# Shanmuk4622/RL-Project-Heist-Architect-Adversarial-Reinforcement-Learning-Framework-CSE4019

Hardware: AMD Instinct MI355X
Metric: Solver env-steps/sec at 20×20, 4096 envs/GPU, 1/2/4/8 MI355X (higher is better)
Workload: dtype f64

## Files before the change

rl-project-heist-architect-adversarial-reinforcement-learning-framework-cse4019_amd/csrc/heist_env.hip:

```cpp
#include <type_traits>
#include <utility>

#include "heist_device.h"
#include "heist_fan_intervals.h"
#include "heist_trig.h"

#pragma clang fp contract(off)

namespace heist {

__constant__ double kSinCosTab[4 * HEIST_SINCOS_TAB_ROWS] = HEIST_SINCOS_TAB_INIT;
constexpr int kTabDoubles = 4 * HEIST_SINCOS_TAB_ROWS;

__device__ __forceinline__ int iabs_(int a) { return a < 0 ? -a : a; }
__device__ __forceinline__ int unpack_r(uint16_t v) { return v & 0xff; }
__device__ __forceinline__ int unpack_c(uint16_t v) { return v >> 8; }

__device__ __forceinline__ double py_mod360(double x) {
  if (x > 0.0 && x < 720.0) return x >= 360.0 ? x - 360.0 : x;
  double r = fmod(x, 360.0);
  if (r != 0.0) {
    if (r < 0.0) r += 360.0;
  } else {
    r = 0.0;
// ... 1976 lines not shown
  float2* uq = reinterpret_cast<float2*>(reinterpret_cast<unsigned char*>(tb) + align16(sizeof(TieBuckets)));
  const int n_chunk = (RC + 63) >> 6;
  const int nvis = (RC + 31) >> 5, WR = (nvis + 4) & ~3;
  uint16_t* togo = reinterpret_cast<uint16_t*>(uq + 128 * W);
  uint32_t* vrow = reinterpret_cast<uint32_t*>(togo + 2 * RC);
  const EnvBase eb = env_base(p, e);

  {
    EmitterRaw raw;
    prefetch<NT>(p, e, eb, L, raw);
    if (t < n_slot) rec[t] = raw;
  }
  for (int i = t; i < path_words; i += NT) L.path[i] = eb.paths[i];
  for (int i = t; i < (int)sizeof(TieBuckets) / 4; i += NT)
    reinterpret_cast<uint32_t*>(tb)[i] = reinterpret_cast<const uint32_t*>(&kTieBuckets_)[i];
  const EnvScalars s = p.scal[e];
  const int tick0 = uni(s.tick);
  int HK = p.max_steps - tick0;
  HK = HK < H ? HK : H;
  if (uni(s.done) || HK < 0) HK = 0;
  const int g = t - mc;
  const bool live_cam = t < s.n_cams, live_guard = g >= 0 && g < s.n_guards;
  bool cached = false;
  uint4 ca = make_uint4(0u, 0u, 0u, 0u), cb = ca;
  auto next_entry = [&](const Guard& gd) {
    int idx = gd.idx, slot = gd.hslot;
    if (gd.len >= 2) {
      idx += gd.step;
      if (idx >= gd.len) idx -= gd.len;
      slot = gd.nslot;
    }
    const uint4* src = reinterpret_cast<const uint4*>(eb.cones + cone_off(g, idx, slot));
    ca = src[0];
    cb = src[1];
  };
  auto take_entry = [&]() {
    Guard gd = as_guard(rec[t]);
    gd.nslot = (uint8_t)(cb.w >> 16);
    rec[t] = __builtin_bit_cast(EmitterRaw, gd);
    uint4* dst = reinterpret_cast<uint4*>(L.cone + 16 * g);
    dst[0] = ca;
    dst[1] = cb;
  };
  __syncthreads();
  if (HK > 0 && live_guard) {
    const Guard gd = as_guard(rec[t]);
    cached = gd.hslot != kUncached;
    if (cached) next_entry(gd);
  }

  const uint32_t cdiv = ((1u << 20) + (uint32_t)C - 1u) / (uint32_t)C;

  for (int k = 1; k <= HK; ++k) {
    Emit E;
    E.kind = -1;
    if (w0) {
      if (live_cam) {
        Cam cm = as_cam(rec[t]);
        cm.heading = py_mod360(cm.heading + cm.speed * 1.0);
        rec[t] = __builtin_bit_cast(EmitterRaw, cm);
        E = cam_emit(cm);
      } else if (live_guard) {
        Guard gd = as_guard(rec[t]);
        const bool moves = gd.len >= 2;
        int nidx = gd.idx;
        if (moves) {
          nidx += gd.step;
          if (nidx >= gd.len) nidx -= gd.len;
        }
        const uint16_t np = moves ? L.path[__umul24((uint32_t)g, (uint32_t)p.max_path) + (uint32_t)nidx] : gd.pos;
        if (cached) {
          if (moves) gd.hslot = gd.nslot;
        } else if (moves) {
          gd.heading = guard_heading_after(p, unpack_r(np) - unpack_r(gd.pos), unpack_c(np) - unpack_c(gd.pos),
                                           gd.heading);
        }
        gd.idx = (int16_t)nidx;
        gd.pos = np;
        rec[t] = __builtin_bit_cast(EmitterRaw, gd);
        E = guard_emit(gd);
        if (cached && !SOLO) take_entry();
      }
      publish_emitters(L, E, n_slot);
    }
    clear_planes<NT>(p, L, gvis, true);
    __syncthreads();
    if (live_guard && E.kind == 1) L.vis[L.at(E.row, E.col)] = 1;
    cast_rays<NT, D, false, true>(smem, L, p.ray_mode, 0, p.half_deg, tb, uq);
    if (SOLO && cached) take_entry();
    stamp_guard_cones<NT>(L, gvis, mc, mg, 0);
    __syncthreads();

    uint32_t* row = vis_out + ((size_t)(k - 1) * N + e) * WR;
    for (int ch = wave; ch < n_chunk; ch += W) {
      const int cell = 64 * ch + lane;
      bool on = false;
      if (cell < RC) {
        const int r = (int)(((uint32_t)cell * cdiv) >> 20), c = cell - r * C;
        const int a = L.at(r, c);
        on = (L.vis[a] | gvis[a]) != 0;
      }
      const unsigned long long m = __ballot(on);
      if (lane < 2 && 2 * ch + lane < WR) row[2 * ch + lane] = (uint32_t)(m >> (32 * lane));
    }
    for (int i = 2 * n_chunk + t; i < WR; i += NT) row[i] = 0u;
    if (w0 && live_guard && cached && k < HK) next_entry(as_guard(rec[t]));
    __syncthreads();
  }

  {
    const int q4 = WR >> 2;
    const uint4 z = make_uint4(0u, 0u, 0u, 0u);
    for (int i = t; i < (H - HK) * q4; i += NT) {
      const int r = HK + i / q4, q = i - (i / q4) * q4;
      reinterpret_cast<uint4*>(vis_out + ((size_t)r * N + e) * WR)[q] = z;
    }
  }
  if (togo_ticks_out)
    for (int k = HK; k < H; ++k) {
      int16_t* trow = togo_ticks_out + ((size_t)k * N + e) * RC;
      for (int x = t; x < RC; x += NT) trow[x] = (int16_t)-1;
    }
  if (HK == 0) {
    for (int x = t; x < RC; x += NT) {
      togo_out[(size_t)e * RC + x] = (int16_t)-1;
      action_out[(size_t)e * RC + x] = (int8_t)-1;
    }
    return;
  }

  __threadfence();
  for (int x = t; x < RC; x += NT) togo[(HK & 1) * RC + x] = (uint16_t)kNone;
  auto load_row = [&](int k) {
    return __hip_atomic_load(vis_out + ((size_t)k * N + e) * WR + (t < nvis ? t : 0), __ATOMIC_RELAXED,
                             __HIP_MEMORY_SCOPE_AGENT);
  };
  __syncthreads();
  {
    const uint32_t w = load_row(HK - 1);
    if (t < nvis) vrow[((HK - 1) & 1) * nvis + t] = w;
  }
  __syncthreads();
  const int vcell = p.vr * C + p.vc;
  for (int k = HK - 1; k >= 0; --k) {
    uint32_t ahead = 0u;
    if (k > 0) ahead = load_row(k - 1);
    const uint32_t* vk = vrow + (k & 1) * nvis;
    const uint16_t* nxt = togo + ((k + 1) & 1) * RC;
    uint16_t* cur = togo + (k & 1) * RC;
    int16_t* trow = togo_ticks_out ? togo_ticks_out + ((size_t)k * N + e) * RC : nullptr;
    for (int x = t; x < RC; x += NT) {
      uint32_t best = kNone;
      int act = -1;
      if (L.grid[x] != kWall) {
        const int r = (int)(((uint32_t)x * cdiv) >> 20), c = x - r * C;
        auto val = [&](int y) -> uint32_t {
          if ((vk[y >> 5] >> (y & 31)) & 1u) return kNone;
          if (y == vcell) return 1u;
          const uint32_t v = nxt[y];
          return v == kNone ? kNone : v + 1u;
        };
        auto moved = [&](bool inside, int y) { return inside && L.grid[y] != kWall ? y : x; };
        best = val(x);
        act = 0;
        uint32_t v = val(moved(r > 0, x - C));
        if (v < best) best = v, act = 1;
        v = val(moved(r + 1 < p.R, x + C));
        if (v < best) best = v, act = 2;
        v = val(moved(c > 0, x - 1));
        if (v < best) best = v, act = 3;
        v = val(moved(c + 1 < C, x + 1));
        if (v < best) best = v, act = 4;
        if (best == kNone) act = -1;
      }
      cur[x] = (uint16_t)best;
      if (trow) trow[x] = (int16_t)(uint16_t)best;
      if (k == 0) {
        togo_out[(size_t)e * RC + x] = (int16_t)(uint16_t)best;
        action_out[(size_t)e * RC + x] = (int8_t)act;
      }
    }
    if (k > 0 && t < nvis) vrow[((k - 1) & 1) * nvis + t] = ahead;
    __syncthreads();
  }
}


__device__ __forceinline__ void lds_dma16(const void* gsrc, uint32_t lds_dst) {
  unsigned keep;
  asm volatile("s_mov_b32 %0, m0\n\ts_mov_b32 m0, %2\n\ts_nop 0\n\tglobal_load_lds_dwordx4 %1, off\n\ts_mov_b32 m0, %0"
               : "=&s"(keep)
               : "v"(gsrc), "s"(lds_dst)
               : "memory");
}

template <int D, int PC>
__device__ __noinline__ void lean_tie_rays(unsigned char* smem, const FanTick* f, int n_tie, uint32_t cam_rc, int n_cams,
                                           const double* hd) {
  const int lane = threadIdx.x;
  for (int b0 = 0; b0 < n_tie; b0 += 64) {
    const int tr = b0 + lane < n_tie ? (int)f->tie[b0 + lane] : -1;
    for (int m = 0; m < n_cams; ++m) {
      Emit E;
      E.hmh = f->hmh;
      E.fov = f->fov;
      E.step = 0.0;
      E.range = f->range;
      E.num_rays = f->num_rays;
      const uint32_t rcm = (uint32_t)__builtin_amdgcn_readlane((int)cam_rc, m);
      E.row = (int)(rcm & 0xffu);
      E.col = (int)(rcm >> 8);
      E.first = 0;
      E.kind = 0;
      E.members = 1;
      if (tr >= 0) exact_ray<D>(smem, E, tr, PC, 0, hd);
    }
  }
}

template <int D, int PC>
__device__ __noinline__ void ivl_tie_rays(unsigned char* smem, int ray, double hmh, double fov, int num_rays,
                                          uint32_t rc, const double* hd) {
  Emit E;
  E.hmh = hmh;
  E.fov = fov;
  E.step = 0.0;
  E.range = kTieMaxRange;
  E.num_rays = num_rays;
  E.row = (int)(rc & 0xffu);
  E.col = (int)(rc >> 8);
  E.first = 0;
  E.kind = 0;
  E.members = 1;
  if (ray >= 0) exact_ray<D>(smem, E, ray, PC, 0, hd);
}

size_t step_multi_lds(const EnvParams& p, int K);
struct LeanStage {
  uint4 off4[128];
  uint2 off2[128];
  int hdr[4];
};

constexpr double kFanUnitsPerDeg = 4294967296.0 / 360.0;
struct IvlTable {
  uint32_t cut[kFanCuts];
  float2 dir[kFanCuts];
  uint8_t idx[368];
};
static_assert(sizeof(IvlTable) % 16 == 0, "copied in 16-byte words");
constexpr IvlTable make_ivl_table() {
  IvlTable t{};
  for (int j = 0; j < kFanCuts; ++j) {
    t.cut[j] = kFanCut[j];
    t.dir[j] = float2{kFanDir[j][0], kFanDir[j][1]};
  }
  for (int d = 0; d < 361; ++d) t.idx[d] = kFanIdx[d];
  return t;
}
__constant__ IvlTable kIvlTable = make_ivl_table();
constexpr size_t kLeanUnion = sizeof(LeanStage) > sizeof(IvlTable) ? sizeof(LeanStage) : sizeof(IvlTable);
struct LeanLds {
  uint8_t* grid;
  uint16_t* path;
  uint8_t* act;
  LeanStage* stg;
  IvlTable* ivl;
  uint4* icam;
  int32_t* icim;
  uint16_t* cone;
  uint16_t* rcone;
  uint8_t* gpl;
  float4* plane2;
};
__host__ __device__ constexpr int lean_gap(int R, int C) { return (R + 2 * kRing) * (C + 2 * kRing) <= 1024 ? 1024 : 2048; }
__host__ __device__ inline size_t lean_carve(unsigned char* smem, int R, int C, int mc, int mg, int mp, int K,
                                             LeanLds* L) {
  size_t o = 3 * (size_t)lean_gap(R, C);
  if (L) L->grid = smem + o;
  o += align16((size_t)R * C);
  if (L) L->path = reinterpret_cast<uint16_t*>(smem + o);
  o += align16(2 * (size_t)mg * mp);
  if (L) L->act = smem + o;
  o += align16((size_t)K);
  if (L) L->stg = reinterpret_cast<LeanStage*>(smem + o);
  if (L) L->ivl = reinterpret_cast<IvlTable*>(smem + o);
  o += align16(kLeanUnion);
  if (L) L->icam = reinterpret_cast<uint4*>(smem + o);
  o += 16 * (size_t)(mc > 0 ? mc : 1);
  if (L) L->icim = reinterpret_cast<int32_t*>(smem + o);
  o += align16(8 * (size_t)(mc > 0 ? mc : 1));
  if (L) L->cone = reinterpret_cast<uint16_t*>(smem + o);
  o += 64 * (size_t)(mg > 0 ? mg : 1);
  if (L) L->rcone = reinterpret_cast<uint16_t*>(smem + o);
  o += 64 * (size_t)(mg > 0 ? mg : 1);
  if (L) L->gpl = smem + o;
  o += align16((size_t)R * C);
  if (L) L->plane2 = reinterpret_cast<float4*>(smem + o);
  o += 4 * (size_t)R * C;
  return o;
}
static size_t lean_lds_bytes(const EnvParams& p, int K) {
  const size_t lean = align16(lean_carve(nullptr, p.R, p.C, p.max_cams, p.max_guards, p.max_path, K, nullptr)) +
                      (p.stamps ? 80 : 0);
  const size_t generic = step_multi_lds(p, K);
  return lean > generic ? lean : generic;
}


struct LeanGuard {
  uint32_t a, b, nslot;
  __device__ int idx() const { return (int)(a & 0xffu); }
  __device__ int step() const { return (int)((a >> 8) & 0xffu); }
  __device__ int len() const { return (int)((a >> 16) & 0xffu); }
  __device__ int hslot() const { return (int)(a >> 24); }
  __device__ uint32_t pos() const { return b & 0xffffu; }
  __device__ uint32_t pos0() const { return b >> 16; }
};

template <int D, bool REC>
__device__ __attribute__((noinline)) void lean_generic_body(EnvParams p, int K, const int64_t* __restrict__ actions,
                                                            obs_out_t<REC>* __restrict__ obs, float* __restrict__ rew,
                                                            double* __restrict__ rew64, uint8_t* __restrict__ done_out,
                                                            int8_t* __restrict__ status_out, int auto_reset,
                                                            unsigned char* smem, int e) {
  step_multi_body<1, D, false, 0, REC>(p, K, actions, obs, rew, rew64, done_out, status_out, auto_reset, smem, e);
}

template <int R_, int C_, bool STAMP = false, int NW = 1, bool REC = false>
__global__ __launch_bounds__(64 * NW) __attribute__((amdgpu_waves_per_eu(4))) void step_lean_kernel(
    EnvParams p, int K, const int64_t* __restrict__ actions, obs_out_t<REC>* __restrict__ obs, float* __restrict__ rew,
    double* __restrict__ rew64, uint8_t* __restrict__ done_out, int8_t* __restrict__ status_out, int auto_reset) {
  constexpr int D = lean_gap(R_, C_);
  constexpr int PC = C_ + 2 * kRing;
  constexpr int RC = R_ * C_;
  constexpr int N4 = RC / 4;
  constexpr int C4 = C_ / 4;
  constexpr int Q = (N4 + 63) / 64;
  constexpr int OFF0 = kRing * PC + kRing;
  static_assert((R_ + 2 * kRing) * PC <= D, "the padded planes fit the 1024-byte gap");
  static_assert(C_ % 4 == 0 && R_ <= 64 && C_ <= 32 && (R_ + 2 * kRing) * PC <= 2048, "lean kernel geometry");
  static_assert(NW == 1 || (NW == 2 && !STAMP && Q % 2 == 0), "two waves: the plain form, even Q");
  constexpr int QW = Q / NW;
  static_assert(!REC || !STAMP, "record output: the plain instances only");
  constexpr int NVIS = (RC + 31) / 32;
  constexpr int RW = (NVIS + 1 + 3) & ~3;
  constexpr int kStores = REC ? QW + 1 + 4 : 3 * QW + 4;
  extern __shared__ __align__(16) unsigned char smem[];
  const int e = block_env(p);
  if (p.prio_mode && p.dispatch_order) {
    const int pr = (int)((uint32_t)p.order[blockIdx.x] >> 24);
    if (pr == 3) __builtin_amdgcn_s_setprio(3);
    else if (pr == 2) __builtin_amdgcn_s_setprio(2);
    else if (pr == 1) __builtin_amdgcn_s_setprio(1);
  }
  const int lane = NW == 1 ? (int)threadIdx.x : (int)(threadIdx.x & 63u);
  const int wid = NW == 1 ? 0 : __builtin_amdgcn_readfirstlane((int)(threadIdx.x >> 6));
  const int tid = threadIdx.x;
  const int N = p.n_envs;
  const int mc = p.max_cams, mg = p.max_guards, n_slot = mc + mg, mp = p.max_path;
  const EnvBase eb = env_base(p, e);
  const FanTick* fan0 = p.fan + p.fan_base;

  EnvScalars s = p.scal[e];
  const int g = lane - mc;
  double heading = 0.0, speed = 0.0;
  uint32_t cam_rc = 0;
  LeanGuard gd{0u, 0u, 0u};
  const bool live_cam = lane < s.n_cams, live_guard = g >= 0 && g < s.n_guards;
  bool cached = false;
  double fovd = 0.0, su = 1.0;
  int32_t im_fx = 0;
  int cam_n = 0;
  bool ivl = false;
  {
    EmitterRaw rec;
    rec.a = make_uint4(0u, 0u, 0u, 0u);
    rec.b = rec.a;
    if (lane < n_slot) {
      const uint4* rs = lane < mc ? reinterpret_cast<const uint4*>(eb.cams + (uint32_t)lane)
                                  : reinterpret_cast<const uint4*>(eb.guards + (uint32_t)g);
      rec.a = rs[0];
      rec.b = rs[1];
    }
    const Cam cm = as_cam(rec);
    const Guard gr = as_guard(rec);
    heading = cm.heading;
    speed = cm.speed;
    cam_rc = (uint32_t)cm.row | ((uint32_t)cm.col << 8);
    cached = live_guard && gr.hslot != kUncached;
    gd.a = (uint32_t)(uint8_t)gr.idx | ((uint32_t)(uint8_t)gr.step << 8) | ((uint32_t)(uint8_t)gr.len << 16) |
           ((uint32_t)gr.hslot << 24);
    gd.b = (uint32_t)gr.pos | ((uint32_t)gr.pos0 << 16);
    gd.nslot = gr.nslot;
    const double f_heading = fan0->heading, f_speed = fan0->speed, f_fov = fan0->fov;
    const int f_rays = fan0->num_rays, f_range = fan0->range, f_uniq = fan0->n_uniq;
    const bool cam_ok = !live_cam || (py_mod360(cm.heading + cm.speed * 1.0) == f_heading && cm.speed == f_speed &&
                                      cm.fov == f_fov && cm.num_rays == f_rays && cm.range == f_range);
    const bool base_ok = p.ray_mode == 0 && !s.done && __ballot(live_guard && !cached) == 0ull;
    const bool fan_ok = p.fan_on && f_uniq >= 0 && f_range == kTieMaxRange && __ballot(!cam_ok) == 0ull;
    const double su_ = (cm.fov / (double)cm.num_rays) * kFanUnitsPerDeg;
    const bool ivl_cam = !live_cam || (cm.range == kTieMaxRange && cm.num_rays >= 1 && cm.fov > 0.0 &&
                                       cm.fov < 170.0 && su_ > 2.0 * (double)kFanMarginAxis + 8.0 &&
                                       su_ >= 2097153.0);
    ivl = base_ok && !fan_ok && p.interval_fans && __ballot(!ivl_cam) == 0ull;
    if (!base_ok || (!fan_ok && !ivl)) {
      if (NW == 2 && wid != 0) return;
      lean_generic_body<D, REC>(p, K, actions, obs, rew, rew64, done_out, status_out, auto_reset, smem, e);
      return;
    }
    if (live_cam) {
      fovd = cm.fov;
      su = su_;
      im_fx = (int32_t)__builtin_rint(4503599627370496.0 / su_);
      cam_n = cm.num_rays;
    }
  }

  LeanLds L;
  const size_t carved = lean_carve(smem, R_, C_, mc, mg, mp, K, &L);
  unsigned long long* st_acc = reinterpret_cast<unsigned long long*>(smem + align16(carved));
  unsigned long long st_last = 0, st_start = 0;
  if (STAMP && lane == 0) {
    st_start = st_last = __builtin_amdgcn_s_memtime();
    for (int j = 0; j < 9; ++j) st_acc[j] = 0;
  }
#define LEAN_STAMP(seg)                                        \
  do {                                                         \
    if (STAMP && lane == 0) {                                  \
      const unsigned long long now_ = __builtin_amdgcn_s_memtime(); \
      st_acc[(seg)] += now_ - st_last;                         \
      st_last = now_;                                          \
    }                                                          \
  } while (0)
  uint8_t* const wall = smem;
  uint8_t* const vis = smem + D;
  const uint32_t base = (uint32_t)(uintptr_t)smem;
  const uint32_t stg_a = (uint32_t)__builtin_amdgcn_readfirstlane((int)(uint32_t)(uintptr_t)L.stg);
  const uint32_t stc_a = (uint32_t)__builtin_amdgcn_readfirstlane((int)(uint32_t)(uintptr_t)L.cone);
  const uint32_t str_a = (uint32_t)__builtin_amdgcn_readfirstlane((int)(uint32_t)(uintptr_t)L.rcone);
  const uint32_t gpl_a = (uint32_t)__builtin_amdgcn_readfirstlane((int)(uint32_t)(uintptr_t)L.gpl);
  static_assert(RC % 16 == 0, "the packed guard plane is cleared in 16-byte words");
  {
    const uint32_t* g4 = reinterpret_cast<const uint32_t*>(p.grid + (size_t)e * RC);
    for (int i = tid; i < N4; i += 64 * NW) reinterpret_cast<uint32_t*>(L.grid)[i] = g4[i];
    const uint8_t* ss = p.stop + (size_t)e * p.stop_bytes;
    for (int i = tid; i < p.stop_bytes; i += 64 * NW) expand_stop(wall, i, ss[i]);
    const int vault = p.vr * C_ + p.vc, qv = vault >> 2;
    for (int q = tid; q < N4; q += 64 * NW) {
      float4 v = reinterpret_cast<const float4*>(p.plane0)[q];
      if (q == qv) patch4(v, vault & 3, p.vault_val);
      L.plane2[q] = v;
    }
  }
  for (int i = tid; i < mg * mp; i += 64 * NW) L.path[i] = eb.paths[i];
  for (int k = tid; k < K; k += 64 * NW) {
    const int64_t a = actions[(size_t)k * N + e];
    L.act[k] = (uint8_t)((a < 0 || a > 4) ? 0 : a);
  }
  __syncthreads();
  uint32_t vwall = 0;
  if (lane < R_)
    for (int c = 0; c < C_; ++c) vwall |= (uint32_t)wall[OFF0 + lane * PC + c] << c;

  auto dma_fan = [&](int k, bool wide) {
    const FanTick* f = fan0 + k;
    lds_dma16(f->off4 + lane, stg_a + (uint32_t)offsetof(LeanStage, off4));
    if (wide) lds_dma16(f->off4 + 64 + lane, stg_a + (uint32_t)offsetof(LeanStage, off4) + 1024u);
    lds_dma16(f->off2 + 2 * lane, stg_a + (uint32_t)offsetof(LeanStage, off2));
    if (lane == 0) lds_dma16(&f->num_rays, stg_a + (uint32_t)offsetof(LeanStage, hdr));
  };
  auto dma_cone = [&](int idx, int slot, uint32_t stage, int par) {
    if (cached) {
      const uint16_t* src = eb.cones + cone_off((uint32_t)g, (uint32_t)idx, (uint32_t)slot);
      const uint32_t dst = stage + (uint32_t)(par * 32 * mg) - 16u * (uint32_t)mc;
      lds_dma16(src, dst);
      lds_dma16(src + 8, dst + 16u * (uint32_t)mg);
    }
  };
  auto dma_next_cone = [&](int par) {
    int idx = gd.idx(), slot = gd.hslot();
    if (gd.len() >= 2) {
      idx += gd.step();
      if (idx >= gd.len()) idx -= gd.len();
      slot = (int)gd.nslot;
    }
    dma_cone(idx, slot, stc_a, par);
    if (auto_reset) dma_cone(0, slot, str_a, par);
  };
  if (wid == 0) dma_next_cone(0);
  if (ivl) {
    for (uint32_t o = 1024u * (uint32_t)wid; o < (uint32_t)sizeof(IvlTable); o += 1024u * NW)
      if (o + 16u * (uint32_t)lane < (uint32_t)sizeof(IvlTable))
        lds_dma16(reinterpret_cast<const unsigned char*>(&kIvlTable) + o + 16u * (uint32_t)lane, stg_a + o);
  } else if (wid == 0) {
    dma_fan(0, true);
  }
  asm volatile("s_waitcnt vmcnt(0)" ::: "memory");
  if (NW == 2) __syncthreads();

  const uint64_t cmask = __ballot(cached);
  auto stamp_cones = [&](const uint16_t* rows, int par) {
    if (lane < RC / 16) reinterpret_cast<uint4*>(L.gpl)[lane] = make_uint4(0u, 0u, 0u, 0u);
    const uint32_t gposv = gd.pos();
    for (int pass = 0; pass * 4 < mg; ++pass) {
      const int i = lane / 15, j = lane - 15 * i;
      const int gs = 4 * pass + i;
      const uint32_t gp = (uint32_t)__shfl((int)gposv, mc + (gs < mg ? gs : 0), 64);
      if (lane < 60 && gs < mg && ((cmask >> (mc + gs)) & 1u)) {
        const uint32_t bits = rows[par * 16 * mg + (j >> 3) * 8 * mg + 8 * gs + (j & 7)] & 0x7fffu;
        if (bits) {
          const uint32_t a0 = gpl_a + (unpack_r((uint16_t)gp) + j - kConeRange) * C_ +
                              (unpack_c((uint16_t)gp) - kConeRange);
          const uint32_t m = bits << (a0 & 3u);
          const uint32_t a = a0 & ~3u;
#pragma unroll
          for (int w = 0; w < 5; ++w) {
            const uint32_t nib = (m >> (4 * w)) & 15u;
            if (nib)
              __hip_atomic_fetch_or(reinterpret_cast<__attribute__((address_space(3))) uint32_t*>(a + 4 * w),
                                    __umul24(nib, 0x204081u) & 0x01010101u, __ATOMIC_RELAXED,
                                    __HIP_MEMORY_SCOPE_WORKGROUP);
          }
        }
      }
    }
  };
  auto march = [&](uint32_t corner, uint4 o4, uint2 o2) {
    const uint32_t ow[6] = {o4.x, o4.y, o4.z, o4.w, o2.x, o2.y};
    uint32_t a[12], w[12];
#pragma unroll
    for (int u = 0; u < 12; ++u) a[u] = corner + ((u & 1) ? (ow[u >> 1] >> 16) : (ow[u >> 1] & 0xffffu));
#pragma unroll
    for (int u = 0; u < 12; ++u) w[u] = lds_ld(a[u]);
    const uint32_t own0 = (ow[0] & 0xffffu) == (uint32_t)OFF0, own1 = (ow[0] >> 16) == (uint32_t)OFF0;
    uint32_t stop = 0;
#pragma unroll
    for (int u = 0; u < 12; ++u) {
      stop = u == 0 ? w[0] : or_b32(stop, w[u]);
      const uint32_t skip = u == 0 ? or_b32(stop, own0) : (u == 1 ? or_b32(stop, own1) : stop);
      lds_st(__umul24(skip, (uint32_t)D) + a[u] + D, 1);
    }
  };
  auto cast_fan = [&](int k, int n_uniq, int n_tie, int par, bool staged_wide) {
#pragma unroll
    for (int z = 0; z < D / 1024; ++z)
      reinterpret_cast<uint4*>(vis)[lane + 64 * z] = make_uint4(0u, 0u, 0u, 0u);
    const FanTick* f = fan0 + k;
    uint4 o4a = make_uint4(0u, 0u, 0u, 0u), o4b = o4a;
    uint2 o2a = make_uint2(0u, 0u), o2b = o2a;
    if (s.n_cams > 0) {
      const bool want_b = n_uniq > 64;
      o4a = L.stg->off4[lane];
      o2a = L.stg->off2[lane];
      if (want_b && staged_wide) {
        o4b = L.stg->off4[64 + lane];
        o2b = L.stg->off2[64 + lane];
      }
      if (want_b && !staged_wide) {
        o4b = f->off4[64 + lane];
        o2b = f->off2[64 + lane];
        asm volatile("" ::"v"(__builtin_bit_cast(u32x4_t, o4a)), "v"(__builtin_bit_cast(u32x2_t, o2a)),
                     "v"(__builtin_bit_cast(u32x4_t, o4b)), "v"(__builtin_bit_cast(u32x2_t, o2b)));
      }
    }
    if (k + 1 < K) {
      asm volatile("s_waitcnt lgkmcnt(0)" ::"v"(__builtin_bit_cast(u32x4_t, o4a)), "v"(__builtin_bit_cast(u32x2_t, o2a)),
                   "v"(__builtin_bit_cast(u32x4_t, o4b)), "v"(__builtin_bit_cast(u32x2_t, o2b))
                   : "memory");
      dma_fan(k + 1, n_uniq > 64);
    }
    if (s.n_cams > 0) {
      for (int m = 0; m < s.n_cams; ++m) {
        const uint32_t rcm = (uint32_t)__builtin_amdgcn_readlane((int)cam_rc, m);
        const uint32_t corner = base + (rcm & 0xffu) * PC + (rcm >> 8);
        if (lane < n_uniq) march(corner, o4a, o2a);
        if (lane + 64 < n_uniq) march(corner, o4b, o2b);
        for (int c0 = 128; c0 < n_uniq; c0 += 64)
          if (lane + c0 < n_uniq) march(corner, f->off4[lane + c0], f->off2[lane + c0]);
      }
      if (n_tie > 0) lean_tie_rays<D, PC>(smem, f, n_tie, cam_rc, s.n_cams, p.half_deg);
    }
    LEAN_STAMP(2);
    stamp_cones(L.cone, par);
  };
  auto wave_join = [&]() {
    if constexpr (NW == 2) asm volatile("s_waitcnt lgkmcnt(0)\n\ts_barrier" ::: "memory");
  };
  auto cast_ivl = [&](int par) {
    wave_join();
#pragma unroll
    for (int z = wid; z < D / 1024; z += NW)
      reinterpret_cast<uint4*>(vis)[lane + 64 * z] = make_uint4(0u, 0u, 0u, 0u);
    const double hmh = heading - fovd / 2.0;
    const double hu = (hmh < 0.0 ? hmh + 360.0 : hmh) * kFanUnitsPerDeg;
    const uint32_t h0v = hu >= 4294967295.0 ? 0xFFFFFFFFu : (uint32_t)hu;
    int cnt = 0, jb = 0;
    if (live_cam) {
      jb = (int)L.ivl->idx[__umulhi(h0v, 360u)] - 1;
      const uint64_t e64 = (uint64_t)h0v + (uint64_t)((double)cam_n * su) + (uint64_t)(kFanMarginAxis + 4);
      const int je = (int)L.ivl->idx[__umulhi((uint32_t)e64, 360u) + 1u] + kFanCuts * (int)(e64 >> 32);
      cnt = je - jb;
      L.icam[lane] = make_uint4(h0v, (uint32_t)jb, (uint32_t)cam_n | (cam_rc << 16), 0u);
      L.icim[lane] = im_fx;
    }
    int total = 0, jo_l = 0, end_l = 0;
    for (int m = 0; m < s.n_cams; ++m) {
      if (lane == m) jo_l = jb - total;
      total += __builtin_amdgcn_readlane(cnt, m);
      if (lane == m) end_l = total;
    }
    auto march_at = [&](uint32_t rc, float2 d) {
      const uint32_t row = rc & 0xffu, col = rc >> 8;
      const uint32_t own = base + (row + kRing) * PC + col + kRing;
      const float mx = __builtin_bit_cast(float, base + col + kRing), my = __builtin_bit_cast(float, row + kRing);
      march_fast<D, 2 * kTieMaxRange, false, false, true>(PC, own, d.x, d.y, mx, my, 2 * kTieMaxRange);
    };
    int mb = 0;
    wave_join();
    for (int q0 = 64 * wid; q0 < total; q0 += 64 * NW) {
      const int q = q0 + lane;
      while (__builtin_amdgcn_readlane(end_l, mb) <= q0) ++mb;
      int c = mb, jo = __builtin_amdgcn_readlane(jo_l, mb);
      for (int m = mb; m + 1 < s.n_cams; ++m) {
        const int em = __builtin_amdgcn_readlane(end_l, m);
        if (em >= q0 + 64) break;
        const int jo_m = __builtin_amdgcn_readlane(jo_l, m + 1);
        if (q >= em) {
          c = m + 1;
          jo = jo_m;
        }
      }
      int j = jo + q;
      j = j < 0 ? j + kFanCuts : (j >= kFanCuts ? j - kFanCuts : j);
      const uint4 cu = L.icam[c];
      const int im = L.icim[c];
      const int n = (int)(cu.z & 0xffffu);
      const int jn = j + 1 == kFanCuts ? 0 : j + 1;
      const uint32_t cut = L.ivl->cut[j], cutn = L.ivl->cut[jn];
      const float2 dj = L.ivl->dir[j];
      const int rel = (int)(cut - cu.x), reln = (int)(cutn - cu.x);
      const int mj = (cut & 0x3FFFFFFFu) ? kFanMarginTie : kFanMarginAxis;
      const int mn = (cutn & 0x3FFFFFFFu) ? kFanMarginTie : kFanMarginAxis;
      const int A = (__mulhi(rel + mj, im) >> 20) + 1;
      const int B = -(__mulhi(mj - rel, im) >> 20);
      const int Bn = -(__mulhi(mn - reln, im) >> 20);
      const int a0 = A > 0 ? A : 0;
      const bool act = q < total;
      const bool safe = act && a0 <= n && a0 < Bn;
      const bool near = act && B < A && B >= 0 && B <= n;
      if (__ballot(near)) {
        const double h_c = __shfl(hmh, c, 64), f_c = __shfl(fovd, c, 64);
        ivl_tie_rays<D, PC>(smem, near ? B : -1, h_c, f_c, n, cu.z >> 16, p.half_deg);
      }
      if (safe) march_at(cu.z >> 16, dj);
    }
    LEAN_STAMP(2);
    if (wid == 0) stamp_cones(L.cone, par);
    wave_join();
  };
  auto cast = [&](int k, int n_uniq, int n_tie, int par, bool staged_wide) {
    if (ivl) {
      cast_ivl(par);
    } else {
      wave_join();
      if (wid == 0) cast_fan(k, n_uniq, n_tie, par, staged_wide);
      wave_join();
    }
  };
  auto read_v1 = [&](uint32_t (&v1)[QW]) {
#pragma unroll
    for (int j = 0; j < QW; ++j) {
      const int q = lane + 64 * (wid * QW + j), qc = q < N4 ? q : N4 - 1, r = qc / C4;
      v1[j] = *reinterpret_cast<const uint32_t*>(vis + OFF0 + r * PC + 4 * (qc - r * C4)) |
              *reinterpret_cast<const uint32_t*>(L.gpl + 4 * qc);
    }
  };

  constexpr uint32_t kOOB = 0x40000000u;
  uint32_t vact = 0;
  bool wide = true;
  for (int k = 0; k < K; ++k) {
    const int par = k & 1;
    if ((k & 63) == 0) vact = k + lane < K ? L.act[k + lane] : 0u;
    asm volatile("s_waitcnt vmcnt(%0)" ::"i"(kStores) : "memory");
    int n_uniq = 0, n_tie = 0;
    if (!ivl && wid == 0) {
      const int2 h = *reinterpret_cast<const int2*>(&L.stg->hdr[2]);
      n_uniq = __builtin_amdgcn_readfirstlane(h.x);
      n_tie = __builtin_amdgcn_readfirstlane(h.y);
    }
    LEAN_STAMP(0);
    const bool staged_wide = wide;
    const bool frozen = s.done != 0;
    double reward = 0.0;
    int status = kAlreadyDone, curr = 0;
    if (!frozen) {
      const int a = __builtin_amdgcn_readlane((int)vact, k & 63);
      const int nr = s.pos_r + (a == 1 ? -1 : (a == 2 ? 1 : 0)), nc = s.pos_c + (a == 3 ? -1 : (a == 4 ? 1 : 0));
      if (nr >= 0 && nr < R_ && nc >= 0 && nc < C_ && !((__builtin_amdgcn_readlane((int)vwall, nr) >> nc) & 1)) {
        s.pos_r = nr;
        s.pos_c = nc;
      }
      status = kRunning;
      curr = iabs_(s.pos_r - p.vr) + iabs_(s.pos_c - p.vc);
      reward = p.r_step;
      reward += (double)(s.prev_dist - curr) * 0.1;
      if (curr <= 3 && s.initial_dist > 3) reward += 0.05 * (double)(3 - curr);
      s.prev_dist = curr;
      if (live_cam) heading = py_mod360(heading + speed * 1.0);
      if (live_guard && gd.len() >= 2) {
        int nidx = gd.idx() + gd.step();
        if (nidx >= gd.len()) nidx -= gd.len();
        const uint32_t np = L.path[__umul24((uint32_t)g, (uint32_t)mp) + (uint32_t)nidx];
        gd.a = (uint32_t)nidx | (gd.a & 0x00ffff00u) | (gd.nslot << 24);
        gd.b = np | (gd.b & 0xffff0000u);
      }
      if (cached && wid == 0) gd.nslot = L.cone[par * 16 * mg + 8 * mg + 8 * g + 7];
      if (k + 1 < K && wid == 0) dma_next_cone(par ^ 1);
      LEAN_STAMP(1);
      cast(k, n_uniq, n_tie, par, staged_wide);
      LEAN_STAMP(3);
    }
    wide = n_uniq > 64;
    uint32_t v1[QW];
    read_v1(v1);
    int done_now = s.done;
    LEAN_STAMP(4);
    if (!frozen) {
      bool seen;
      if constexpr (NW == 1) {
        const int sol = s.pos_r * C_ + s.pos_c, qs = sol >> 2;
        uint32_t vq = v1[0];
#pragma unroll
        for (int j = 1; j < Q; ++j) vq = (qs >> 6) == j ? v1[j] : vq;
        const uint32_t qv = (uint32_t)__builtin_amdgcn_readlane((int)vq, qs & 63);
        seen = ((qv >> (8 * (sol & 3))) & 0xffu) != 0u;
      } else {
        seen = (vis[OFF0 + s.pos_r * PC + s.pos_c] | L.gpl[s.pos_r * C_ + s.pos_c]) != 0;
      }
      if (seen) {
        s.detected = 1;
        reward += p.r_detect;
        s.done = 1;
        status = kDetected;
      }
      if (s.pos_r == p.vr && s.pos_c == p.vc) {
        s.vault_reached = 1;
        reward += p.r_vault;
        s.done = 1;
        status = kVaultReached;
      }
      s.tick += 1;
      if (s.tick >= p.max_steps) {
        s.done = 1;
        status = kTimeout;
        double frac = 1.0 - (double)curr / (double)(s.initial_dist > 1 ? s.initial_dist : 1);
        if (frac < 0.0) frac = 0.0;
        reward += frac * 2.0;
      }
      done_now = s.done;
    }
    LEAN_STAMP(5);
    if (auto_reset && done_now) {
      const bool moved = __ballot(live_guard && gd.pos() != gd.pos0()) != 0ull;
      reset_solver(p, s);
      if (live_guard) {
        gd.a &= ~0xffu;
        gd.b = (gd.b & 0xffff0000u) | gd.pos0();
      }
      if (cached && wid == 0) gd.nslot = L.rcone[par * 16 * mg + 8 * mg + 8 * g + 7];
      if (moved) {
        wave_join();
        if (wid == 0) stamp_cones(L.rcone, par);
        wave_join();
        read_v1(v1);
      }
      if (k + 1 < K && wid == 0) dma_next_cone(par ^ 1);
    }
    LEAN_STAMP(6);
    asm volatile("" ::: "memory");
    if constexpr (REC) {
      uint32_t* o = obs + ((size_t)k * N + e) * RW;
      const __amdgpu_buffer_rsrc_t rs = __builtin_amdgcn_make_buffer_rsrc(o, (short)0, 4 * RW, 0x00020000);
#pragma unroll
      for (int j = 0; j < QW; ++j) {
        const int q = lane + 64 * (wid * QW + j);
        uint32_t w = (q < N4 ? vis_nibble(v1[j]) : 0u) << (4 * (lane & 7));
        w = or8_lanes(w);
        const int wi = q >> 3;
        __builtin_amdgcn_raw_buffer_store_b32(w, rs, (lane & 7) == 0 && wi < NVIS ? 4 * wi : (int)kOOB, 0, 0);
      }
      __builtin_amdgcn_raw_buffer_store_b32(lane == 0 ? (uint32_t)s.pos_r | ((uint32_t)s.pos_c << 8) : 0u, rs,
                                            wid == 0 && lane < RW - NVIS ? 4 * (NVIS + lane) : (int)kOOB, 0, 0);
    } else {
      constexpr int pol = 2;
      float* o = obs + ((size_t)k * N + e) * 3 * RC;
      const __amdgpu_buffer_rsrc_t rs = __builtin_amdgcn_make_buffer_rsrc(o, (short)0, 12 * RC, 0x00020000);
      const int sol = s.pos_r * C_ + s.pos_c, qs = sol >> 2;
      const int vault = p.vr * C_ + p.vc;
  #pragma unroll
      for (int j = 0; j < QW; ++j) {
        const int q = lane + 64 * (wid * QW + j);
        const bool in = q < N4;
        const int qc = in ? q : N4 - 1;
        const uint32_t b = *reinterpret_cast<const uint32_t*>(L.grid + 4 * qc);
        obs_put(rs, pol, in ? 16 * q : (int)kOOB,
                make_float4((float)(b & 0xff) * 0.2f, (float)((b >> 8) & 0xff) * 0.2f,
                            (float)((b >> 16) & 0xff) * 0.2f, (float)(b >> 24) * 0.2f));
        const uint32_t v = v1[j];
        obs_put(rs, pol, in ? 16 * (N4 + q) : (int)kOOB,
                make_float4((float)(v & 0xff), (float)((v >> 8) & 0xff), (float)((v >> 16) & 0xff), (float)(v >> 24)));
        float4 c2 = L.plane2[qc];
        const bool pl = q == qs && sol != vault;
        const int m = sol & 3;
        c2.x = pl && m == 0 ? 1.0f + c2.x : c2.x;
        c2.y = pl && m == 1 ? 1.0f + c2.y : c2.y;
        c2.z = pl && m == 2 ? 1.0f + c2.z : c2.z;
        c2.w = pl && m == 3 ? 1.0f + c2.w : c2.w;
        obs_put(rs, pol, in ? 16 * (2 * N4 + q) : (int)kOOB, c2);
      }
    }
    const uint32_t ko = (uint32_t)((size_t)k * N + e);
    const int l0 = lane == 0 && wid == 0 ? 0 : (int)kOOB;
    __builtin_amdgcn_raw_buffer_store_b32(__builtin_bit_cast(uint32_t, (float)reward),
                                          __builtin_amdgcn_make_buffer_rsrc(rew + ko, (short)0, 4, 0x00020000), l0, 0, 0);
    __builtin_amdgcn_raw_buffer_store_b64(__builtin_bit_cast(u32x2_t, __builtin_bit_cast(uint64_t, reward)),
                                          __builtin_amdgcn_make_buffer_rsrc(rew64 ? rew64 + ko : rew64, (short)0,
                                                                            rew64 ? 8 : 0, 0x00020000),
                                          l0, 0, 0);
    __builtin_amdgcn_raw_buffer_store_b8((uint8_t)done_now,
                                         __builtin_amdgcn_make_buffer_rsrc(done_out + ko, (short)0, 1, 0x00020000), l0,
                                         0, 0);
    __builtin_amdgcn_raw_buffer_store_b8((uint8_t)(int8_t)status,
                                         __builtin_amdgcn_make_buffer_rsrc(status_out + ko, (short)0, 1, 0x00020000),
                                         l0, 0, 0);
    LEAN_STAMP(7);
  }
  if (STAMP && lane == 0) {
    unsigned long long* q = p.stamps + (size_t)e * p.multi_waves * 16;
    for (int j = 0; j < 9; ++j) q[j] = st_acc[j];
    q[9] = __builtin_amdgcn_s_memtime() - st_start;
    q[10] = st_start;
    q[11] = (unsigned)__builtin_amdgcn_s_getreg((31 << 11) | 4);
    q[12] = (unsigned)__builtin_amdgcn_s_getreg((31 << 11) | 20);
  }
#undef LEAN_STAMP
  if (wid != 0) return;
  if (lane == 0) p.scal[e] = s;
  if (live_cam) eb.cams[(uint32_t)lane].heading = heading;
  if (live_guard) {
    const uint4 c2 = reinterpret_cast<const uint4*>(eb.cones + cone_off(g, gd.idx(), gd.hslot()))[2];
    Guard* gp = eb.guards + (uint32_t)g;
    gp->heading = __builtin_bit_cast(double, ((uint64_t)c2.y << 32) | c2.x);
    gp->idx = (int16_t)gd.idx();
    gp->pos = (uint16_t)gd.pos();
    gp->hslot = (uint8_t)gd.hslot();
    gp->nslot = (uint8_t)gd.nslot;
  }
}

template <int W, int D>
__global__ __launch_bounds__(64 * W) __attribute__((amdgpu_waves_per_eu(kStepOcc))) void reset_kernel(EnvParams p, const uint8_t* __restrict__ mask,
                                                        float* __restrict__ obs) {
  constexpr int NT = 64 * W;
  extern __shared__ __align__(16) unsigned char smem[];
  const int e = block_env(p);
  const int t = threadIdx.x;
  if (mask && !mask[e]) return;
  const EnvLds L = carve<D>(smem, p.R, p.C, p.max_cams + p.max_guards, 0, W, p.max_guards);
  const EnvBase eb = env_base(p, e);
  EmitterRaw raw;
  prefetch<NT>(p, e, eb, L, raw);
  EnvScalars s = p.scal[e];
  const int mc = p.max_cams, n_slot = p.max_cams + p.max_guards;
  clear_vis<NT>(p, L);
  __syncthreads();
  reset_solver(p, s);
  Emit E;
  E.kind = -1;
  if (t < s.n_cams) {
    E = cam_emit(as_cam(raw));
  } else if (t >= mc && t - mc < s.n_guards) {
    Guard gd = as_guard(raw);
    gd.idx = 0;
    gd.pos = gd.pos0;
    Guard* gp = eb.guards + (uint32_t)(t - mc);
    gp->idx = 0;
    gp->pos = gd.pos0;
    if (gd.hslot != kUncached) {
      stage_guard_cone(p, e, L, t - mc, gd, false);
      gp->nslot = (uint8_t)L.cone[16 * (t - mc) + 15];
    }
    E = guard_emit(gd);
  }
  publish_emitters(L, E, n_slot);
  raycast_pass<NT, D>(p, e, smem, L, n_slot, mc);
  write_obs<NT>(p, e, s, L, 0, obs);
  if (t == 0) p.scal[e] = s;
}


__device__ __forceinline__ void write_stop_map(const EnvParams& p, int e, const uint8_t* g, int lane, int stride) {
  const int R = p.R, C = p.C, PC = C + 2 * kRing, nb = (R + 2 * kRing) * PC;
  uint8_t* stp = p.stop + (size_t)e * p.stop_bytes;
  for (int j = lane; j < p.stop_bytes; j += stride) {
    uint32_t bits = 0;
    for (int k = 0; k < 8; ++k) {
      const int i = 8 * j + k;
      const int pr = i / PC;
      const int r = pr - kRing, c = i - pr * PC - kRing;
      const bool out = i >= nb || (unsigned)r >= (unsigned)R || (unsigned)c >= (unsigned)C;
      if (out || g[r * C + c] == kWall) bits |= 1u << k;
    }
    stp[j] = (uint8_t)bits;
  }
}

int stop_map_bytes(int R, int C) { return (int)align16((size_t)(padded_bytes(R, C) + 7) / 8); }

__device__ bool bfs_wave(uint64_t pass, int sr, int sc, int gr, int gc) {
  const int lane = threadIdx.x & 63;
  if (sr == gr && sc == gc) return true;
  uint64_t reach = lane == sr ? (1ull << sc) : 0ull;
  const uint64_t goal = lane == gr ? (1ull << gc) : 0ull;
  for (int it = 0; it < kMaxDim * kMaxDim; ++it) {
    const uint64_t up = __shfl(reach, lane > 0 ? lane - 1 : 0);
    const uint64_t dn = __shfl(reach, lane < 63 ? lane + 1 : 63);
    const uint64_t nb = (reach | (reach << 1) | (reach >> 1) | (lane > 0 ? up : 0ull) | (lane < 63 ? dn : 0ull)) & pass;
    const uint64_t nxt = reach | nb;
    const bool hit = __any((nxt & goal) != 0ull);
    const bool grew = __any(nxt != reach);
    reach = nxt;
    if (hit) return true;
    if (!grew) return false;
  }
  return false;
}

__global__ __launch_bounds__(64) void set_layout_kernel(EnvParams p, int max_walls, const int32_t* __restrict__ wall_rc,
                                                         const int32_t* __restrict__ n_walls,
                                                         const double* __restrict__ cam_params,
                                                         const int32_t* __restrict__ n_cams,
                                                         const int32_t* __restrict__ guard_paths,
                                                         const int32_t* __restrict__ guard_meta,
                                                         const double* __restrict__ guard_fov,
                                                         const int32_t* __restrict__ n_guards,
                                                         const int32_t* __restrict__ budget,
                                                         const uint8_t* __restrict__ mask,
                                                         uint8_t* __restrict__ valid_out) {
  __shared__ uint8_t g[kMaxDim * kMaxDim];
  __shared__ int cnt[4];
  const int e = blockIdx.x;
  if (mask && !mask[e]) return;
  const int lane = threadIdx.x;
  const int R = p.R, C = p.C;
  for (int i = lane; i < p.RC; i += 64) {
    const int r = i / C, c = i - (i / C) * C;
    g[i] = (r == 0 || r == R - 1 || c == 0 || c == C - 1) ? kWall : kEmpty;
  }
  __syncthreads();
  if (lane == 0) {
    g[p.sr * C + p.sc] = kStart;
    g[p.vr * C + p.vc] = kVault;
    const int total = budget[e];
    int spent = 0, nw = 0, nc = 0, ng = 0;
    auto placeable = [&](int r, int c) {
      return r > 0 && r < R - 1 && c > 0 && c < C - 1 && g[r * C + c] == kEmpty;
    };
    const int wn = min(n_walls[e], max_walls);
    for (int i = 0; i < wn; ++i) {
      const int r = wall_rc[((size_t)e * max_walls + i) * 2], c = wall_rc[((size_t)e * max_walls + i) * 2 + 1];
      if (placeable(r, c) && total - spent >= 1) {
        spent += 1;
        g[r * C + c] = kWall;
        ++nw;
      }
    }
    const int cn = min(n_cams[e], p.max_cams);
    for (int i = 0; i < cn; ++i) {
      const double* cp = cam_params + ((size_t)e * p.max_cams + i) * 6;
      const int r = (int)cp[0], c = (int)cp[1];
      if (placeable(r, c) && total - spent >= 3) {
        spent += 3;
        Cam cm;
        cm.fov = cp[2]; cm.heading = cp[3]; cm.speed = cp[4];
        cm.row = (int16_t)r; cm.col = (int16_t)c; cm.range = (int16_t)cp[5];
        cm.num_rays = (int16_t)num_rays_for(cm.fov);
        p.cams[(size_t)e * p.max_cams + nc] = cm;
        g[r * C + c] = kCamera;
        ++nc;
      }
    }
    const int gn = min(n_guards[e], p.max_guards);
    for (int i = 0; i < gn; ++i) {
      const int32_t* gm = guard_meta + ((size_t)e * p.max_guards + i) * 3;
      const int len = min(gm[0], p.max_path);
      if (len > 0 && total - spent >= 5) {
        spent += 5;
        const int32_t* src = guard_paths + ((size_t)e * p.max_guards + i) * p.max_path * 2;
        uint16_t* dst = p.paths + ((size_t)e * p.max_guards + ng) * p.max_path;
        for (int k = 0; k < len; ++k) {
          const int pr = min(max(src[2 * k], 0), R - 1), pc = min(max(src[2 * k + 1], 0), C - 1);
          dst[k] = (uint16_t)pack_rc(pr, pc);
        }
        Guard gd;
        gd.fov = guard_fov[(size_t)e * p.max_guards + i];
        gd.heading = 0.0;
        gd.idx = 0;
        int st = gm[1] % len;
        if (st < 0) st += len;
        gd.step = (int16_t)st;
        gd.len = (int16_t)len;
        gd.range = (int16_t)gm[2];
        gd.num_rays = (int16_t)num_rays_for(gd.fov);
        gd.pos = dst[0];
        gd.pos0 = dst[0];
        gd.hslot = kUncached;
        gd.nslot = kUncached;
        p.guards[(size_t)e * p.max_guards + ng] = gd;
        g[unpack_r(dst[0]) * C + unpack_c(dst[0])] = kGuard;
        ++ng;
      }
    }
    cnt[0] = nw; cnt[1] = nc; cnt[2] = ng; cnt[3] = spent;
  }
  __syncthreads();
  uint64_t m = 0;
  if (lane < R)
    for (int c = 0; c < C; ++c)
      if (g[lane * C + c] != kWall) m |= 1ull << c;
  const bool ok = bfs_wave(m, p.sr, p.sc, p.vr, p.vc);
  uint8_t* dst = p.grid + (size_t)e * p.RC;
  for (int i = lane; i < p.RC; i += 64) dst[i] = g[i];
  write_stop_map(p, e, g, lane, 64);
  if (lane == 0) {
    EnvScalars* s = p.scal + e;
    s->n_walls = cnt[0];
    s->n_cams = cnt[1];
    s->n_guards = cnt[2];
    s->spent = cnt[3];
    valid_out[e] = ok ? 1 : 0;
  }
}

template <int D>
__global__ __launch_bounds__(64) void guard_cone_kernel(EnvParams p, const uint8_t* __restrict__ mask) {
  extern __shared__ __align__(16) unsigned char smem[];
  __shared__ double heads[kConeSlots];
  __shared__ uint8_t arr[kConePath];
  __shared__ int n_heads;
  const int e = blockIdx.x, g = blockIdx.y;
  const int lane = threadIdx.x;
  if (mask && !mask[e]) return;
  if (g >= p.scal[e].n_guards) return;
  Guard* gp = p.guards + (size_t)e * p.max_guards + g;
  const Guard gd = *gp;
  const int len = gd.len;
  if (!p.guard_cones || len < 1 || len > kConePath || gd.range < 0 || gd.range > kConeRange) return;
  const int R = p.R, C = p.C;
  const EnvLds L = carve<D>(smem, R, C, 1, kConePath, 1);
  const uint8_t* ss = p.stop + (size_t)e * p.stop_bytes;
  for (int i = lane; i < p.stop_bytes; i += 64) expand_stop(L.wall, i, ss[i]);
  if (lane < len) L.path[lane] = p.paths[((size_t)e * p.max_guards + g) * p.max_path + lane];
  __syncthreads();
  if (lane == 0) {
    int nh = 1;
    heads[0] = gd.heading;
    for (int j = 0; j < len; ++j) {
      int i0 = j - gd.step;
      if (i0 < 0) i0 += len;
      const int dr = unpack_r(L.path[j]) - unpack_r(L.path[i0]), dc = unpack_c(L.path[j]) - unpack_c(L.path[i0]);
      if (len < 2 || (dr == 0 && dc == 0)) {
        arr[j] = kUncached;
        continue;
      }
      const double h = guard_heading_after(p, dr, dc, 0.0);
      int k = 0;
      while (k < nh && heads[k] != h) ++k;
      if (k == nh) {
        if (nh == kConeSlots) {
          nh = 0;
          break;
        }
        heads[nh++] = h;
      }
      arr[j] = (uint8_t)k;
    }
    n_heads = nh;
  }
  __syncthreads();
  const int nh = n_heads;
  if (nh == 0) return;
  uint32_t* v4 = reinterpret_cast<uint32_t*>(L.vis);
  for (int st = 0; st < len * nh; ++st) {
    const int i = st / nh, h = st - i * nh;
    for (int q = lane; q < (padded_bytes(R, C) + 3) / 4; q += 64) v4[q] = 0u;
    __syncthreads();
    Emit E;
    E.hmh = heads[h] - gd.fov / 2.0;
    E.fov = gd.fov;
    E.step = 0.0;
    E.row = unpack_r(L.path[i]);
    E.col = unpack_c(L.path[i]);
    E.range = gd.range;
    E.num_rays = gd.num_rays;
    E.first = 0;
    E.kind = 1;
    E.members = 1;
    for (int ray = lane; ray <= E.num_rays; ray += 64) exact_ray<D>(smem, E, ray, L.PC, 0, p.half_deg);
    __syncthreads();
    if (lane < kConeEntry) {
      uint32_t bits = 0;
      if (lane >= 16) {
        const uint64_t hb = __builtin_bit_cast(uint64_t, heads[h]);
        bits = lane < 20 ? (uint32_t)(hb >> (16 * (lane - 16))) & 0xffffu : (lane == 20 ? (uint32_t)L.path[i] : 0u);
      } else if (lane < 2 * kConeRange + 1) {
        const int rr = E.row + lane - kConeRange;
        if ((unsigned)rr < (unsigned)R)
          for (int j = 0; j < 2 * kConeRange + 1; ++j) {
            const int cc = E.col + j - kConeRange;
            if ((unsigned)cc < (unsigned)C && (L.vis[L.at(rr, cc)] || (rr == E.row && cc == E.col))) bits |= 1u << j;
          }
      } else {
        int i2 = i + gd.step;
        if (i2 >= len) i2 -= len;
        bits = (len >= 2 && arr[i2] != kUncached) ? arr[i2] : (uint32_t)h;
      }
      p.cones[cone_entry(p, e, g, i, h) + lane] = (uint16_t)bits;
    }
    __syncthreads();
  }
  if (lane == 0) {
    const int i2 = gd.step < len ? gd.step : 0;
    gp->hslot = 0;
    gp->nslot = (len >= 2 && arr[i2] != kUncached) ? arr[i2] : 0;
  }
}

__global__ __launch_bounds__(64) void bfs_kernel(const int32_t* __restrict__ grid, int R, int C, int sr, int sc, int gr,
                                                  int gc, uint8_t* __restrict__ out) {
  const int e = blockIdx.x;
  const int lane = threadIdx.x;
  const int32_t* g = grid + (size_t)e * R * C;
  uint64_t m = 0;
  if (lane < R)
    for (int c = 0; c < C; ++c)
      if (g[lane * C + c] != kWall) m |= 1ull << c;
  const bool ok = bfs_wave(m, sr, sc, gr, gc);
  if (lane == 0) out[e] = ok ? 1 : 0;
}

template <int D>
__global__ __launch_bounds__(64) void cones_kernel(int R, int C, const uint8_t* __restrict__ walls,
                                                    const int32_t* __restrict__ meta, const double* __restrict__ params,
                                                    uint8_t* __restrict__ out, int ray_mode) {
  extern __shared__ __align__(16) unsigned char smem[];
  const int e = blockIdx.x;
  const int lane = threadIdx.x;
  const int RC = R * C;
  const EnvLds L = carve<D>(smem, R, C, 1, 0, 1);
  for (int i = lane; i < RC; i += 64) L.grid[i] = walls[(size_t)e * RC + i] ? kWall : kEmpty;
// ... 479 lines not shown
```

Before: 804.3 million.

## Overlap lean kernel prologue loads and DMA grid/plane copies into LDS

Hoists the global loads for fan tick, stop bits, paths, actions, emitter records and env scalars to the kernel entry so they are issued together under one wait. The grid and base observation plane are now copied into LDS with direct buffer-to-LDS DMA overlapping the fan DMA, and the vault cell is patched afterwards. One generic-path barrier is replaced by a waitcnt plus s_barrier for the two-wave form. Extra stamp slots are added for profiling entry and loop-start times. The aim is to cut prologue latency per env; it adds register pressure and ordering risk around the LDS DMA.

```diff
diff --git a/rl-project-heist-architect-adversarial-reinforcement-learning-framework-cse4019_amd/csrc/heist_env.hip b/rl-project-heist-architect-adversarial-reinforcement-learning-framework-cse4019_amd/csrc/heist_env.hip
--- a/rl-project-heist-architect-adversarial-reinforcement-learning-framework-cse4019_amd/csrc/heist_env.hip
+++ b/rl-project-heist-architect-adversarial-reinforcement-learning-framework-cse4019_amd/csrc/heist_env.hip
@@ -2302,7 +2302,7 @@
 }
 static size_t lean_lds_bytes(const EnvParams& p, int K) {
   const size_t lean = align16(lean_carve(nullptr, p.R, p.C, p.max_cams, p.max_guards, p.max_path, K, nullptr)) +
-                      (p.stamps ? 80 : 0);
+                      (p.stamps ? 96 : 0);
   const size_t generic = step_multi_lds(p, K);
   return lean > generic ? lean : generic;
 }
@@ -2347,6 +2347,10 @@
   constexpr int RW = (NVIS + 1 + 3) & ~3;
   constexpr int kStores = REC ? QW + 1 + 4 : 3 * QW + 4;
   extern __shared__ __align__(16) unsigned char smem[];
+  const unsigned long long st_entry = STAMP ? __builtin_amdgcn_s_memtime() : 0ull;
+  const FanTick* fan0 = p.fan + p.fan_base;
+  const double f_heading = fan0->heading, f_speed = fan0->speed, f_fov = fan0->fov;
+  const int f_rays = fan0->num_rays, f_range = fan0->range, f_uniq = fan0->n_uniq;
   const int e = block_env(p);
   if (p.prio_mode && p.dispatch_order) {
     const int pr = (int)((uint32_t)p.order[blockIdx.x] >> 24);
@@ -2360,10 +2364,37 @@
   const int N = p.n_envs;
   const int mc = p.max_cams, mg = p.max_guards, n_slot = mc + mg, mp = p.max_path;
   const EnvBase eb = env_base(p, e);
-  const FanTick* fan0 = p.fan + p.fan_base;
-
-  EnvScalars s = p.scal[e];
+  constexpr int NT = 64 * NW;
+
+  const uint32_t* ss4 = reinterpret_cast<const uint32_t*>(p.stop + (size_t)e * p.stop_bytes);
+  const int n_stop4 = p.stop_bytes >> 2, n_path = mg * mp;
+  uint32_t stop_v = 0u, path_v = 0u;
+  int64_t act_v = 0;
+  if (tid < n_stop4) stop_v = ss4[tid];
+  if (tid < n_path) path_v = eb.paths[tid];
+  if (tid < K) act_v = actions[(size_t)tid * N + e];
   const int g = lane - mc;
+  EmitterRaw rec;
+  rec.a = make_uint4(0u, 0u, 0u, 0u);
+  rec.b = rec.a;
+  if (lane < n_slot) {
+    const uint4* rs = lane < mc ? reinterpret_cast<const uint4*>(eb.cams + (uint32_t)lane)
+                                : reinterpret_cast<const uint4*>(eb.guards + (uint32_t)g);
+    rec.a = rs[0];
+    rec.b = rs[1];
+  }
+  EnvScalars s;
+  {
+    static_assert(sizeof(EnvScalars) == 48, "three 16-byte loads");
+    const u32x4_t* sp = reinterpret_cast<const u32x4_t*>(p.scal + e);
+    u32x4_t s0 = sp[0], s1 = sp[1], s2 = sp[2];
+    asm volatile("s_waitcnt vmcnt(0)" : "+v"(s0), "+v"(s1), "+v"(s2)::"memory");
+    s.pos_r = uni((int)s0[0]), s.pos_c = uni((int)s0[1]), s.tick = uni((int)s0[2]), s.done = uni((int)s0[3]);
+    s.detected = uni((int)s1[0]), s.vault_reached = uni((int)s1[1]);
+    s.prev_dist = uni((int)s1[2]), s.initial_dist = uni((int)s1[3]);
+    s.n_cams = uni((int)s2[0]), s.n_guards = uni((int)s2[1]), s.n_walls = uni((int)s2[2]), s.spent = uni((int)s2[3]);
+  }
+  const uint32_t pa_v = path_v | ((uint32_t)((act_v < 0 || act_v > 4) ? 0 : act_v) << 16);
   double heading = 0.0, speed = 0.0;
   uint32_t cam_rc = 0;
   LeanGuard gd{0u, 0u, 0u};
@@ -2374,15 +2405,6 @@
   int cam_n = 0;
   bool ivl = false;
   {
-    EmitterRaw rec;
-    rec.a = make_uint4(0u, 0u, 0u, 0u);
-    rec.b = rec.a;
-    if (lane < n_slot) {
-      const uint4* rs = lane < mc ? reinterpret_cast<const uint4*>(eb.cams + (uint32_t)lane)
-                                  : reinterpret_cast<const uint4*>(eb.guards + (uint32_t)g);
-      rec.a = rs[0];
-      rec.b = rs[1];
-    }
     const Cam cm = as_cam(rec);
     const Guard gr = as_guard(rec);
     heading = cm.heading;
@@ -2393,8 +2415,6 @@
            ((uint32_t)gr.hslot << 24);
     gd.b = (uint32_t)gr.pos | ((uint32_t)gr.pos0 << 16);
     gd.nslot = gr.nslot;
-    const double f_heading = fan0->heading, f_speed = fan0->speed, f_fov = fan0->fov;
-    const int f_rays = fan0->num_rays, f_range = fan0->range, f_uniq = fan0->n_uniq;
     const bool cam_ok = !live_cam || (py_mod360(cm.heading + cm.speed * 1.0) == f_heading && cm.speed == f_speed &&
                                       cm.fov == f_fov && cm.num_rays == f_rays && cm.range == f_range);
     const bool base_ok = p.ray_mode == 0 && !s.done && __ballot(live_guard && !cached) == 0ull;
@@ -2404,7 +2424,7 @@
                                        cm.fov < 170.0 && su_ > 2.0 * (double)kFanMarginAxis + 8.0 &&
                                        su_ >= 2097153.0);
     ivl = base_ok && !fan_ok && p.interval_fans && __ballot(!ivl_cam) == 0ull;
-    if (!base_ok || (!fan_ok && !ivl)) {
+    if (__builtin_amdgcn_readfirstlane(!base_ok || (!fan_ok && !ivl))) {
       if (NW == 2 && wid != 0) return;
       lean_generic_body<D, REC>(p, K, actions, obs, rew, rew64, done_out, status_out, auto_reset, smem, e);
       return;
@@ -2424,6 +2444,7 @@
   if (STAMP && lane == 0) {
     st_start = st_last = __builtin_amdgcn_s_memtime();
     for (int j = 0; j < 9; ++j) st_acc[j] = 0;
+    st_acc[10] = st_entry;
   }
 #define LEAN_STAMP(seg)                                        \
   do {                                                         \
@@ -2440,28 +2461,7 @@
   const uint32_t stc_a = (uint32_t)__builtin_amdgcn_readfirstlane((int)(uint32_t)(uintptr_t)L.cone);
   const uint32_t str_a = (uint32_t)__builtin_amdgcn_readfirstlane((int)(uint32_t)(uintptr_t)L.rcone);
   const uint32_t gpl_a = (uint32_t)__builtin_amdgcn_readfirstlane((int)(uint32_t)(uintptr_t)L.gpl);
-  static_assert(RC % 16 == 0, "the packed guard plane is cleared in 16-byte words");
-  {
-    const uint32_t* g4 = reinterpret_cast<const uint32_t*>(p.grid + (size_t)e * RC);
-    for (int i = tid; i < N4; i += 64 * NW) reinterpret_cast<uint32_t*>(L.grid)[i] = g4[i];
-    const uint8_t* ss = p.stop + (size_t)e * p.stop_bytes;
-    for (int i = tid; i < p.stop_bytes; i += 64 * NW) expand_stop(wall, i, ss[i]);
-    const int vault = p.vr * C_ + p.vc, qv = vault >> 2;
-    for (int q = tid; q < N4; q += 64 * NW) {
-      float4 v = reinterpret_cast<const float4*>(p.plane0)[q];
-      if (q == qv) patch4(v, vault & 3, p.vault_val);
-      L.plane2[q] = v;
-    }
-  }
-  for (int i = tid; i < mg * mp; i += 64 * NW) L.path[i] = eb.paths[i];
-  for (int k = tid; k < K; k += 64 * NW) {
-    const int64_t a = actions[(size_t)k * N + e];
-    L.act[k] = (uint8_t)((a < 0 || a > 4) ? 0 : a);
-  }
-  __syncthreads();
-  uint32_t vwall = 0;
-  if (lane < R_)
-    for (int c = 0; c < C_; ++c) vwall |= (uint32_t)wall[OFF0 + lane * PC + c] << c;
+  static_assert(RC % 16 == 0, "the packed guard plane is cleared, the grid copied in 16-byte words");
 
   auto dma_fan = [&](int k, bool wide) {
     const FanTick* f = fan0 + k;
@@ -2496,7 +2496,38 @@
   } else if (wid == 0) {
     dma_fan(0, true);
   }
+  {
+    const uint32_t grid_a = (uint32_t)__builtin_amdgcn_readfirstlane((int)(uint32_t)(uintptr_t)L.grid);
+    const uint32_t pl2_a = (uint32_t)__builtin_amdgcn_readfirstlane((int)(uint32_t)(uintptr_t)L.plane2);
+    const uint8_t* gsrc = p.grid + (size_t)e * RC;
+    const unsigned char* psrc = reinterpret_cast<const unsigned char*>(p.plane0);
+#pragma unroll
+    for (uint32_t o = 1024u * (uint32_t)wid; o < (uint32_t)RC; o += 1024u * NW)
+      if (o + 16u * (uint32_t)lane < (uint32_t)RC) lds_dma16(gsrc + o + 16u * (uint32_t)lane, grid_a + o);
+#pragma unroll
+    for (uint32_t o = 1024u * (uint32_t)wid; o < 4u * (uint32_t)RC; o += 1024u * NW)
+      if (o + 16u * (uint32_t)lane < 4u * (uint32_t)RC) lds_dma16(psrc + o + 16u * (uint32_t)lane, pl2_a + o);
+  }
+  auto put_stop = [&](int i, uint32_t v) {
+#pragma unroll
+    for (int j = 0; j < 4; ++j) expand_stop(wall, 4 * i + j, (v >> (8 * j)) & 0xffu);
+  };
+  auto put_act = [&](int k, int64_t a) { L.act[k] = (uint8_t)((a < 0 || a > 4) ? 0 : a); };
+  if (tid < n_stop4) put_stop(tid, stop_v);
+  if (tid < n_path) L.path[tid] = (uint16_t)pa_v;
+  if (tid < K) L.act[tid] = (uint8_t)(pa_v >> 16);
+  for (int i = tid + NT; i < n_stop4; i += NT) put_stop(i, ss4[i]);
+  for (int i = tid + NT; i < n_path; i += NT) L.path[i] = eb.paths[i];
+  for (int k = tid + NT; k < K; k += NT) put_act(k, actions[(size_t)k * N + e]);
+  if constexpr (NW == 2) asm volatile("s_waitcnt lgkmcnt(0)\n\ts_barrier" ::: "memory");
+  uint32_t vwall = 0;
+  if (lane < R_)
+    for (int c = 0; c < C_; ++c) vwall |= (uint32_t)wall[OFF0 + lane * PC + c] << c;
   asm volatile("s_waitcnt vmcnt(0)" ::: "memory");
+  {
+    const int vault = p.vr * C_ + p.vc;
+    if (lane == 0 && wid == ((vault >> 8) & (NW - 1))) reinterpret_cast<float*>(L.plane2)[vault] = p.vault_val;
+  }
   if (NW == 2) __syncthreads();
 
   const uint64_t cmask = __ballot(cached);
@@ -2680,6 +2711,7 @@
   constexpr uint32_t kOOB = 0x40000000u;
   uint32_t vact = 0;
   bool wide = true;
+  if (STAMP && lane == 0) st_acc[11] = __builtin_amdgcn_s_memtime();
   for (int k = 0; k < K; ++k) {
     const int par = k & 1;
     if ((k & 63) == 0) vact = k + lane < K ? L.act[k + lane] : 0u;
@@ -2844,8 +2876,9 @@
     q[10] = st_start;
     q[11] = (unsigned)__builtin_amdgcn_s_getreg((31 << 11) | 4);
     q[12] = (unsigned)__builtin_amdgcn_s_getreg((31 << 11) | 20);
-  }
-#undef LEAN_STAMP
+    q[13] = st_acc[10];
+    q[14] = st_acc[11];
+  }
   if (wid != 0) return;
   if (lane == 0) p.scal[e] = s;
   if (live_cam) eb.cams[(uint32_t)lane].heading = heading;
@@ -2858,6 +2891,8 @@
     gp->hslot = (uint8_t)gd.hslot();
     gp->nslot = (uint8_t)gd.nslot;
   }
+  if (STAMP && lane == 0) (p.stamps + (size_t)e * p.multi_waves * 16)[15] = __builtin_amdgcn_s_memtime();
+#undef LEAN_STAMP
 }
 
 template <int W, int D>
```

After: 799.5 million. About the same (-0.6%).
